# confluentinc/quickstart-streaming-agents

Measured on NVIDIA H100. Metric: rag_queries_per_sec_10Mx1536_top10, higher is better.
Workload: dtype bf16

## Files before the change

quickstart-streaming-agents_b200/csrc/sa_api.cu:

```cuda
#include "../../include/sa_api.h"
#include "sa_aux.cuh"
#include "sa_scan.cuh"

#include <cuda.h>
#include <cuda_runtime.h>
#include <dlfcn.h>
#include <nccl.h>

#include <algorithm>
#include <cstdarg>
#include <cstddef>
#include <cstdio>
#include <cstring>
#include <string>
#include <vector>

namespace {

thread_local char g_err[512] = "";

int fail(int rc, const char* fmt, ...) {
  va_list ap;
  va_start(ap, fmt);
  vsnprintf(g_err, sizeof g_err, fmt, ap);
// ... 278 lines not shown
    if (cg == 1 && kl == 16) return launch_scan<1, 16, sa::kModeProd, sa::kEpiSub>(tq, tc, p, grid, st);
    if (cg == 1 && kl == 32) return launch_scan<1, 32, sa::kModeProd, sa::kEpiSub>(tq, tc, p, grid, st);
    if (cg == 2 && kl == 16) return launch_scan<2, 16, sa::kModeProd, sa::kEpiSub>(tq, tc, p, grid, st);
    if (cg == 2 && kl == 32) return launch_scan<2, 32, sa::kModeProd, sa::kEpiSub>(tq, tc, p, grid, st);
    return fail(SA_ERR_ARG, "no scan instantiation for cta_group %d list %d", cg, kl);
  }
  if (mode == sa::kModeDots) {
    if (cg == 1) return launch_scan<1, 16, sa::kModeDots>(tq, tc, p, grid, st);
    return launch_scan<2, 16, sa::kModeDots>(tq, tc, p, grid, st);
  }
  if (mode == sa::kModeProf) {
    if (cg == 1 && kl == 16) return launch_scan<1, 16, sa::kModeProf>(tq, tc, p, grid, st);
    if (cg == 2 && kl == 16) return launch_scan<2, 16, sa::kModeProf>(tq, tc, p, grid, st);
    return fail(SA_ERR_ARG, "the profiling build of the scan exists for 16-entry lists only");
  }
  if (cg == 1 && kl == 16) return launch_scan<1, 16, sa::kModeProd>(tq, tc, p, grid, st);
  if (cg == 1 && kl == 32) return launch_scan<1, 32, sa::kModeProd>(tq, tc, p, grid, st);
  if (cg == 2 && kl == 16) return launch_scan<2, 16, sa::kModeProd>(tq, tc, p, grid, st);
  if (cg == 2 && kl == 32) return launch_scan<2, 32, sa::kModeProd>(tq, tc, p, grid, st);
  return fail(SA_ERR_ARG, "no scan instantiation for cta_group %d list %d", cg, kl);
}

int choose_cg(const sa_engine* e, int nq) {
  if (e->opt_cta_group == 1 || e->opt_cta_group == 2) return e->opt_cta_group;
  return nq > 128 ? 2 : 1;
}

bool is_pinned(const void* p) {
  cudaPointerAttributes a;
  if (cudaPointerGetAttributes(&a, p) != cudaSuccess) {
// ... 30 lines not shown
              const sa::Filter* filters = nullptr) {
  if (nq <= 0 || nq > e->max_batch) return fail(SA_ERR_CAPACITY, "nq %d outside [1, max_batch %d]", nq, e->max_batch);
  if (k <= 0 || k > e->max_k) return fail(SA_ERR_ARG, "k %d outside [1, max_k %d]", k, e->max_k);
  if (!q_bf16 || !out_score || !out_idx) return fail(SA_ERR_ARG, "null buffer");
  if (reinterpret_cast<uintptr_t>(q_bf16) % 16) return fail(SA_ERR_ARG, "query buffer must be 16-byte aligned");
  SA_ON_DEVICE(e->device);

  const int kl = e->opt_list_len ? e->opt_list_len : (k <= 16 ? 16 : 32);
  if (k > kl) return fail(SA_ERR_ARG, "k %d needs candidate lists longer than list_len %d", k, kl);
  const int64_t n_rows = e->n_rows;
  const int num_tiles = static_cast<int>((n_rows + sa::kBlockN - 1) / sa::kBlockN);
  const int cg = choose_cg(e, nq);
  std::vector<LaunchPlan> plan = plan_search(e->num_sms, e->opt_max_launch_qblocks, nq, cg, std::max(num_tiles, 1));
  if (static_cast<int>(plan.size()) > kMaxLaunches)
    return fail(SA_ERR_CAPACITY, "batch needs %zu scan launches (max %d)", plan.size(), kMaxLaunches);
  const int mode = e->opt_profile ? sa::kModeProf : sa::kModeProd;
  const int epi = (e->sim == SA_SIM_EUCLIDEAN ? sa::kEpiSub : sa::kEpiMul) | (filters != nullptr ? sa::kEpiFilt : 0);
  const float eps_rel = scan_eps_rel(e->dim);

  SA_CUDA(cudaStreamWaitEvent(st, e->scratch_free, 0));
  if (e->scratch_dirty) {
    int rc = zero_scan_scratch(e, st);
    if (rc) return rc;
    e->scratch_dirty = false;
  }
  sa_engine::Timing& tm = e->ring[e->n_searches % kTimingRing];
  tm.launches = 0;
  tm.kernels = 0;
  SA_CUDA(cudaEventRecord(tm.ev_total[0], st));
  e->scratch_dirty = true;
  int min_tl = sa::kMaxLanes;
// ... 162 lines not shown
  const double n = static_cast<double>(n_rows), d = e->dim, b = nq;
  tm.bytes = plan.size() * (n * d * 2.0 + n * 4.0) + b * d * 2.0 + b * k * 8.0;
  tm.flops = 2.0 * b * n * d;
  e->n_searches += 1;
  return SA_OK;
}

}

namespace {
template <int kKL>
void run_list(const float* score, const int32_t* row, int n, const float* floor_after, float* out_sc, int32_t* out_id,
              float* out_drop) {
  sa::TopList<kKL> L;
  L.init(nullptr);
  float ones[sa::kChunk];
  for (int j = 0; j < sa::kChunk; ++j) ones[j] = 1.0f;
  for (int c0 = 0; c0 < n; c0 += sa::kChunk) {
    float v[sa::kChunk];
    for (int j = 0; j < sa::kChunk; ++j) {
      const int i = c0 + j;
      v[j] = i < n ? score[i] : NAN;
      if (i < n && floor_after && floor_after[i] > -INFINITY) L.apply_shared(sa::float_to_key(floor_after[i]));
    }
    sa::chunk_process<kKL>(L, v, ones, c0);
  }
  for (int i = 0; i < kKL; ++i) {
    out_sc[i] = L.sc[i];
    out_id[i] = L.id[i] >= 0 ? row[L.id[i]] : -1;
  }
  if (out_drop) *out_drop = L.drop;
}
}

extern "C" {

static_assert(sizeof(sa_filter) == sizeof(sa::Filter) && offsetof(sa_filter, all_of) == offsetof(sa::Filter, all_of) &&
                  offsetof(sa_filter, none_of) == offsetof(sa::Filter, none_of) &&
                  offsetof(sa_filter, any_of) == offsetof(sa::Filter, any_of),
              "sa_filter and sa::Filter must share one layout");
// ... 951 lines not shown
  }
  if (!strcmp(name, "presample")) {
    if (value < -1 || value > 4096) return fail(SA_ERR_ARG, "presample must be in [-1, 4096]");
    e->opt_presample = static_cast<int>(value);
    return SA_OK;
  }
  if (!strcmp(name, "force_fix")) {
    e->opt_force_fix = value ? 1 : 0;
    return SA_OK;
  }
  if (!strcmp(name, "count_fix")) {
    e->opt_count_fix = value ? 1 : 0;
    return SA_OK;
  }
  if (!strcmp(name, "profile")) {
    e->opt_profile = value ? 1 : 0;
    return SA_OK;
  }
  if (!strcmp(name, "share_thresholds")) {
    e->opt_share_thresholds = value ? 1 : 0;
    return SA_OK;
  }
  if (!strcmp(name, "window_bound")) {
    e->opt_window_bound = value ? 1 : 0;
    return SA_OK;
  }
  if (!strcmp(name, "list_len")) {
    if (value != 0 && value != 16 && value != 32) return fail(SA_ERR_ARG, "list_len must be 0, 16 or 32");
    e->opt_list_len = static_cast<int>(value);
    return SA_OK;
  }
// ... 191 lines not shown
```

quickstart-streaming-agents_b200/csrc/sa_scan.cuh:

```cuda
#pragma once
#include "sa_aux.cuh"
#include "sm90_ptx.cuh"
#include <cmath>
#include <cstring>

namespace sa {

constexpr int kBlockM = 128;
constexpr int kBlockN = 256;
constexpr int kHalfN = kWgmmaN;
constexpr int kBlockK = 64;
constexpr int kUmmaK = 16;
constexpr int kScanThreads = 384;
constexpr int kProducerRegs = 40;
constexpr int kConsumerRegs = 232;
constexpr int kChunk = 32;
constexpr int kStagingLd = kHalfN + 4;
constexpr int kWin = 16;
constexpr int kWinWarmTiles = 16;

constexpr int kModeProd = 0;
constexpr int kModeDots = 1;
constexpr int kModeProf = 2;

constexpr int kEpiMul = 0;
constexpr int kEpiSub = 1;
constexpr int kEpiFilt = 2;

template <int kCG, bool kFilt = false>
struct ScanCfg {
  static constexpr int kStages = 3;
  static constexpr int kBRows = kBlockN / kCG;
  static constexpr uint32_t kABytes = kBlockM * kBlockK * 2;
  static constexpr uint32_t kBBytes = kBlockN * kBlockK * 2;
  static constexpr uint32_t kHalfBBytes = kHalfN * kBlockK * 2;
  static constexpr uint32_t kStageBytes = kABytes + kBBytes;
  static constexpr uint32_t kStagingBytes = kBlockM * kStagingLd * sizeof(float);
  static constexpr uint32_t kIcBytes = 4 * kBlockN * sizeof(float);
  static constexpr uint32_t kBarBytes = 2 * kStages * 8;
  static constexpr uint32_t kTagBytes = kFilt ? 4 * kBlockN * sizeof(unsigned long long) : 0;
  static constexpr uint32_t kSmemBytes = kStages * kStageBytes + kStagingBytes + kIcBytes + kBarBytes + kTagBytes + 1024;
  static_assert(kSmemBytes <= 227 * 1024, "H100 allows 227 KB of shared memory per block");
  static_assert(!kFilt || kSmemBytes == 228400, "filtered scan: the unfiltered 220 208 B plus 8 KB of tags");
};

struct ScanProf {
  long long prod_wait_empty;
  long long mma_wait_full;
  long long mma_wait_tempty;
  long long epi_wait_tfull;
  long long epi_busy;
  long long epi_slow_chunks;
  long long total;
  long long tiles;
};

struct ScanParams {
  const float* row_term;
// ... 138 lines not shown
      sc[i] = -INFINITY;
      id[i] = -1;
    }
    thr = thr_floor = published = drop = -INFINITY;
    nxt_key = 0u;
    slot = shared_slot;
  }
  __host__ __device__ __forceinline__ void apply_shared(unsigned key) {
    if (key != 0u) {
      thr_floor = max_nn(thr_floor, float_below(key_to_float(key)));
      thr = max_nn(thr, thr_floor);
    }
  }
};

template <int kKL, int kEpi = kEpiMul>
__host__ __device__ __forceinline__ bool chunk_process(TopList<kKL>& L, float (&v)[kChunk], const float (&w)[kChunk],
                                                       int row_base) {
  auto reduce = [&]() {
    float g[8];
#ifdef __CUDA_ARCH__
#pragma unroll
#endif
    for (int i = 0; i < 8; ++i)
      g[i] = max_nn(max_nn(v[4 * i + 0], v[4 * i + 1]), max_nn(v[4 * i + 2], v[4 * i + 3]));
    return max_nn(max_nn(max_nn(g[0], g[1]), max_nn(g[2], g[3])), max_nn(max_nn(g[4], g[5]), max_nn(g[6], g[7])));
  };
#ifdef __CUDA_ARCH__
#pragma unroll
#endif
  for (int i = 0; i < kChunk; ++i) {
    if constexpr (kEpi == kEpiSub)
      v[i] -= w[i];
    else
      v[i] *= w[i];
  }
  float m = reduce();
  if (!(m > L.thr)) {
    L.drop = max_nn(L.drop, m);
    return false;
  }
  do {
    int pos = kChunk - 1;
#ifdef __CUDA_ARCH__
#pragma unroll
#endif
    for (int j = kChunk - 2; j >= 0; --j) pos = (v[j] == m) ? j : pos;
    float sj = m;
    if (m == 0.f) {
#ifdef __CUDA_ARCH__
#pragma unroll
// ... 2 lines not shown
    }
#ifdef __CUDA_ARCH__
#pragma unroll
#endif
    for (int j = 0; j < kChunk; ++j) v[j] = (j == pos) ? -INFINITY : v[j];
    L.drop = max_nn(L.drop, L.sc[kKL - 1]);
    list_insert<kKL>(L.sc, L.id, sj, row_base + pos);
    L.thr = max_nn(L.sc[kKL - 1], L.thr_floor);
    m = reduce();
  } while (m > L.thr);
  L.drop = max_nn(L.drop, m);
  return true;
}

#ifdef __CUDACC__
template <int kKL, int kMode, int kEpi>
__device__ __forceinline__ int epilogue_half(TopList<kKL>& L, const float* srow, const float* ic, int row0,
                                             float* dbg_row, const unsigned long long* tg = nullptr,
                                             const Filter* fp = nullptr) {
  int slow = 0;
  float v[kChunk], w[kChunk];
#pragma unroll 1
  for (int c = 0; c < kHalfN / kChunk; ++c) {
    unsigned pass = 0u;
    if constexpr ((kEpi & kEpiFilt) != 0) {
      const Filter F = *fp;
#pragma unroll
      for (int j = 0; j < kChunk; ++j) pass |= filter_pass(tg[c * kChunk + j], F) ? (1u << j) : 0u;
    }
    const float4* s4 = reinterpret_cast<const float4*>(srow + c * kChunk);
    const float4* w4 = reinterpret_cast<const float4*>(ic + c * kChunk);
#pragma unroll
    for (int i = 0; i < kChunk / 4; ++i) {
      const float4 x = s4[i], y = w4[i];
      v[4 * i + 0] = x.x;
      v[4 * i + 1] = x.y;
      v[4 * i + 2] = x.z;
      v[4 * i + 3] = x.w;
      w[4 * i + 0] = y.x;
      w[4 * i + 1] = y.y;
      w[4 * i + 2] = y.z;
      w[4 * i + 3] = y.w;
    }
    if constexpr ((kEpi & kEpiFilt) != 0) {
      const float qnan = __int_as_float(0x7fc00000);
#pragma unroll
      for (int j = 0; j < kChunk; ++j) w[j] = ((pass >> j) & 1u) ? w[j] : qnan;
    }
    if constexpr (kMode == kModeDots) {
      if (dbg_row != nullptr) {
#pragma unroll
        for (int j = 0; j < kChunk; ++j) dbg_row[c * kChunk + j] = v[j];
      }
    }
    slow += chunk_process<kKL, kEpi & 1>(L, v, w, row0 + c * kChunk) ? 1 : 0;
    __syncwarp();
  }
  return slow;
}

template <int kCG, int kKL, int kMode, int kEpi = kEpiMul>
__global__ void __launch_bounds__(kScanThreads, 1)
sa_scan_kernel(const __grid_constant__ CUtensorMap tmap_q, const __grid_constant__ CUtensorMap tmap_c,
               const ScanParams p) {
  constexpr bool kFilt = (kEpi & kEpiFilt) != 0;
  using Cfg = ScanCfg<kCG, kFilt>;
  constexpr int kStages = Cfg::kStages;
  constexpr int kRowsPerQb = kBlockM * kCG;
  constexpr bool kProf = (kMode == kModeProf);

  extern __shared__ uint8_t smem_raw[];
  const uint32_t smem_base = (smem_u32(smem_raw) + 1023u) & ~1023u;
  uint8_t* smem_gen = smem_raw + (smem_base - smem_u32(smem_raw));

  float* staging = reinterpret_cast<float*>(smem_gen + kStages * Cfg::kStageBytes);
  float* icbuf = reinterpret_cast<float*>(smem_gen + kStages * Cfg::kStageBytes + Cfg::kStagingBytes);
  const uint32_t bar_base = smem_base + kStages * Cfg::kStageBytes + Cfg::kStagingBytes + Cfg::kIcBytes;
  auto full_bar = [&](int s) { return bar_base + 8u * s; };
  auto empty_bar = [&](int s) { return bar_base + 8u * (kStages + s); };
  auto a_smem = [&](int s) { return smem_base + s * Cfg::kStageBytes; };
  auto b_smem = [&](int s) { return smem_base + s * Cfg::kStageBytes + Cfg::kABytes; };
  const uint32_t tag_base = bar_base + Cfg::kBarBytes;

  const int warp = threadIdx.x >> 5;
  const int lane = threadIdx.x & 31;
  const uint32_t rank = (kCG == 2) ? cluster_ctarank() : 0u;
  const int TL = p.tl_count;
  const int nqb = p.nqb;
  struct Walk {
    int qb, tl, tiles;
  };
  auto walk_of = [&]() {
// ... 70 lines not shown
          }
        }
        if (lockstep) st_relaxed_gpu(p.lane_progress + tl * nqb + qb, tile_no + 1);
      }
      if constexpr (kProf) {
        p.prof[blockIdx.x].prod_wait_empty = waited;
        p.prof[blockIdx.x].tiles = tile_no;
      }
    }
  } else {
    setmaxnreg_inc<kConsumerRegs>();
    const Walk w = walk_of();
    const int qb = w.qb, tl = w.tl, walk_tiles = w.tiles;
    const int g = warp / 4 - 1;
    const int wt = threadIdx.x & 127;
    const bool epi = (warp & 3) < 2;
    const int ew = 2 * g + (warp & 3);
    const int et = 64 * g + wt;
    const bool signaller = wt == 0;
    const uint32_t named_bar = 1 + g;
    float* ic = icbuf + ew * kBlockN;
    float* stg = staging + 64 * g * kStagingLd;
    const int query = qb * kRowsPerQb + static_cast<int>(rank) * kBlockM + et;
    const bool own_query = epi && query < p.nq;
    TopList<kKL> L;
    L.init((p.thr_shared != nullptr && own_query) ? p.thr_shared + query : nullptr);

    constexpr float kPast = ((kEpi & 1) == kEpiSub) ? -1.f : 0.f;
    float4 nx0 = make_float4(0.f, 0.f, 0.f, 0.f), nx1 = nx0;
    auto fetch_ic = [&](int t) {
      const long long r0 = static_cast<long long>(t) * kBlockN + 8 * lane;
      const float4* src = reinterpret_cast<const float4*>(p.row_term + r0);
      if (r0 + 8 <= p.n_rows) {
        nx0 = __ldg(src);
        nx1 = __ldg(src + 1);
      } else {
        float x[8];
#pragma unroll
        for (int j = 0; j < 8; ++j) x[j] = (r0 + j < p.n_rows) ? __ldg(p.row_term + r0 + j) : kPast;
        nx0 = make_float4(x[0], x[1], x[2], x[3]);
        nx1 = make_float4(x[4], x[5], x[6], x[7]);
      }
    };
    if (epi && tl < walk_tiles) fetch_ic(tl * p.tile_stride);
    auto fetch_tags = [&](int t) {
      const long long r0 = static_cast<long long>(t) * kBlockN + 8 * lane;
      const uint32_t dst = tag_base + static_cast<uint32_t>((ew * kBlockN + 8 * lane) * sizeof(unsigned long long));
#pragma unroll
      for (int j = 0; j < 4; ++j) {
        const long long left = p.n_rows - (r0 + 2 * j);
        const uint32_t bytes = left >= 2 ? 16u : (left == 1 ? 8u : 0u);
        cp_async_16(dst + 16u * j, p.row_tags + (bytes != 0u ? r0 + 2 * j : 0), bytes);
      }
    };
    if constexpr (kFilt) {
      if (epi && tl < walk_tiles) fetch_tags(tl * p.tile_stride);
    }

    const bool win_on = p.lane2 != nullptr && TL >= kWin && own_query;
    const size_t win_stride = static_cast<size_t>(p.nqb) * kRowsPerQb;
    unsigned* const win_q = win_on ? p.lane2 + query : nullptr;
    float pub2 = -INFINITY;
    unsigned nx2[kWin] = {};
    bool have2 = false;

    const uint64_t a_desc0 = make_kmajor_sw128_desc(a_smem(0) + g * (64 * kBlockK * 2));
    const uint64_t b_desc0 = make_kmajor_sw128_desc(b_smem(0));
    constexpr uint64_t kStageDesc = Cfg::kStageBytes >> 4;
    constexpr uint64_t kHalfBDesc = Cfg::kHalfBBytes >> 4;
    int stage = 0;
    uint32_t phase = 0;
    long long w_full = 0, w_stage = 0, w_mma = 0, busy = 0, slow_chunks = 0;
    for (int ti = tl; ti < walk_tiles; ti += TL) {
      const int t = ti * p.tile_stride;
      int slow = 0;
      if (epi) {
        if (have2) {
          const unsigned kb = window_bound<kKL>(nx2);
          L.nxt_key = kb > L.nxt_key ? kb : L.nxt_key;
          have2 = false;
        }
        L.apply_shared(L.nxt_key);
        const float qnan = __int_as_float(0x7fc00000);
        auto sc = [&](float x) {
          if constexpr ((kEpi & 1) == kEpiSub)
            return x >= 0.f ? x : qnan;
          else
            return x > 0.f ? x : qnan;
        };
        float4* dst = reinterpret_cast<float4*>(ic + 8 * lane);
        dst[0] = make_float4(sc(nx0.x), sc(nx0.y), sc(nx0.z), sc(nx0.w));
        dst[1] = make_float4(sc(nx1.x), sc(nx1.y), sc(nx1.z), sc(nx1.w));
        __syncwarp();
      }
#pragma unroll
      for (int i = 0; i < kWin; ++i) nx2[i] = 0u;
      float* dbg_row = nullptr;
      if constexpr (kMode == kModeDots) {
        if (own_query && p.dbg_dots != nullptr && t == p.dbg_tile) dbg_row = p.dbg_dots + static_cast<size_t>(query) * kBlockN;
      }
      float acc0[64], acc1[64];
      int prev_stage = -1;
      for (int kb = 0; kb < p.num_kb; ++kb) {
        if constexpr (kProf) {
          const long long c0 = clock64();
          mbar_wait(full_bar(stage), phase, static_cast<uint32_t>(p.wait_hint_ns));
          w_full += clock64() - c0;
        } else {
          mbar_wait(full_bar(stage), phase, static_cast<uint32_t>(p.wait_hint_ns));
        }
        wgmma_fence();
        wgmma_fence_operands(acc0);
        wgmma_fence_operands(acc1);
#pragma unroll
        for (int k = 0; k < kBlockK / kUmmaK; ++k) {
          const uint64_t a_desc = a_desc0 + stage * kStageDesc + 2u * k;
          const uint64_t b_desc = b_desc0 + stage * kStageDesc + 2u * k;
          wgmma_m64n128k16_bf16(acc0, a_desc, b_desc, (kb | k) != 0 ? 1u : 0u);
          wgmma_m64n128k16_bf16(acc1, a_desc, b_desc + kHalfBDesc, (kb | k) != 0 ? 1u : 0u);
        }
        wgmma_commit();
        wgmma_fence_operands(acc0);
        wgmma_fence_operands(acc1);
        if (prev_stage >= 0) {
          wgmma_wait<1>();
          if (signaller) {
            mbar_arrive(empty_bar(prev_stage));
            if constexpr (kCG == 2) mbar_arrive_cluster(empty_bar(prev_stage), rank ^ 1u);
          }
        }
        prev_stage = stage;
        if (++stage == kStages) {
          stage = 0;
          phase ^= 1u;
        }
      }
      long long c0 = 0;
      if constexpr (kProf) c0 = clock64();
      wgmma_wait<0>();
      wgmma_fence_operands(acc0);
      wgmma_fence_operands(acc1);
      if (signaller) {
        mbar_arrive(empty_bar(prev_stage));
        if constexpr (kCG == 2) mbar_arrive_cluster(empty_bar(prev_stage), rank ^ 1u);
      }
      if constexpr (kProf) w_mma += clock64() - c0;
      if (epi && ti + TL < walk_tiles) fetch_ic((ti + TL) * p.tile_stride);
      auto stage_and_score = [&](const float (&acc)[64], int h) {
        long long c1 = 0;
        if constexpr (kProf) c1 = clock64();
        named_bar_sync(named_bar, 128);
#pragma unroll
        for (int j = 0; j < 16; ++j) {
          const int r = 16 * (wt >> 5) + ((wt & 31) >> 2);
          const int col = 8 * j + 2 * (wt & 3);
          *reinterpret_cast<float2*>(stg + r * kStagingLd + col) = make_float2(acc[4 * j + 0], acc[4 * j + 1]);
          *reinterpret_cast<float2*>(stg + (r + 8) * kStagingLd + col) = make_float2(acc[4 * j + 2], acc[4 * j + 3]);
        }
        named_bar_sync(named_bar, 128);
        long long c2 = 0;
        if constexpr (kProf) c2 = clock64();
        if constexpr (kFilt) {
          if (epi && h == 0) {
            cp_async_wait_all();
            __syncwarp();
          }
        }
        if constexpr (kFilt) {
          const unsigned long long* tg =
              reinterpret_cast<const unsigned long long*>(smem_gen + (tag_base - smem_base)) + ew * kBlockN;
          if (epi)
            slow += epilogue_half<kKL, kMode, kEpi>(L, stg + wt * kStagingLd, ic + h * kHalfN, t * kBlockN + h * kHalfN,
                                                    dbg_row != nullptr ? dbg_row + h * kHalfN : nullptr, tg + h * kHalfN,
                                                    p.filters + (own_query ? query : 0));
        } else if (epi) {
          slow += epilogue_half<kKL, kMode, kEpi>(L, stg + wt * kStagingLd, ic + h * kHalfN, t * kBlockN + h * kHalfN,
                                                  dbg_row != nullptr ? dbg_row + h * kHalfN : nullptr);
        }
        if constexpr (kProf) {
          w_stage += c2 - c1;
          busy += clock64() - c2;
        }
      };
      stage_and_score(acc0, 0);
      stage_and_score(acc1, 1);
      if constexpr (kFilt) {
        if (epi && ti + TL < walk_tiles) {
          __syncwarp();
          fetch_tags((ti + TL) * p.tile_stride);
        }
      }
      if constexpr (kProf) slow_chunks += slow;
      if (epi) {
        if (L.slot != nullptr) {
          if (L.sc[kKL - 1] > L.published) {
            L.published = L.sc[kKL - 1];
            atomicMax(L.slot, float_to_key(L.published));
          }
          L.nxt_key = ld_relaxed_gpu_u32(L.slot);
        }
        if (p.lane2 != nullptr && TL >= kWin) {
          const bool fetch = (ti - tl) / TL < kWinWarmTiles || __any_sync(0xffffffffu, slow > 0);
          if (win_on) {
            if (L.sc[1] > pub2) {
              pub2 = L.sc[1];
              st_relaxed_gpu_u32(win_q + static_cast<size_t>(tl) * win_stride, float_to_key(pub2));
            }
// ... 15 lines not shown

    if (own_query) {
      const size_t o = (static_cast<size_t>(blockIdx.x) * kBlockM + et) * kKL;
      float4* ps = reinterpret_cast<float4*>(p.part_score + o);
      int4* pi = reinterpret_cast<int4*>(p.part_idx + o);
#pragma unroll
      for (int i = 0; i < kKL / 4; ++i) {
        ps[i] = make_float4(L.sc[4 * i], L.sc[4 * i + 1], L.sc[4 * i + 2], L.sc[4 * i + 3]);
        pi[i] = make_int4(L.id[4 * i], L.id[4 * i + 1], L.id[4 * i + 2], L.id[4 * i + 3]);
      }
      p.part_drop[static_cast<size_t>(blockIdx.x) * kBlockM + et] = L.drop;
    }
    if constexpr (kProf) {
      if (g == 0 && signaller) {
        p.prof[blockIdx.x].mma_wait_full = w_full;
        p.prof[blockIdx.x].mma_wait_tempty = w_stage;
        p.prof[blockIdx.x].epi_wait_tfull = w_mma;
        p.prof[blockIdx.x].epi_busy = busy;
        p.prof[blockIdx.x].epi_slow_chunks = slow_chunks;
      }
    }
  }

  __syncthreads();
  if (p.dbg_times != nullptr && threadIdx.x == 0) p.dbg_times[2 * blockIdx.x + 1] = globaltimer_ns();
  if constexpr (kProf) {
    if (threadIdx.x == 0) p.prof[blockIdx.x].total = clock64() - t_start;
  }
  if constexpr (kCG == 2) cluster_sync_all();
}
#endif

}
```

quickstart-streaming-agents_b200/csrc/sm90_ptx.cuh:

```cuda
#pragma once
#include <cstdint>
#include <cuda.h>

namespace sa {

#ifndef SA_WATCHDOG_CYCLES
#define SA_WATCHDOG_CYCLES (4000000000ll)
#endif

__device__ __forceinline__ uint32_t smem_u32(const void* p) {
  return static_cast<uint32_t>(__cvta_generic_to_shared(p));
}
__device__ __forceinline__ uint32_t cluster_ctarank() {
  uint32_t r;
  asm volatile("mov.u32 %0, %%cluster_ctarank;" : "=r"(r));
  return r;
}

__device__ __forceinline__ void mbar_init(uint32_t bar, uint32_t count) {
  asm volatile("mbarrier.init.shared::cta.b64 [%0], %1;" ::"r"(bar), "r"(count) : "memory");
}
__device__ __forceinline__ void fence_mbar_init() {
  asm volatile("fence.mbarrier_init.release.cluster;" ::: "memory");
}
// ... 32 lines not shown
      : "r"(bar), "r"(parity), "r"(hint_ns)
      : "memory");
  return ok != 0;
}
__device__ __forceinline__ void mbar_wait(uint32_t bar, uint32_t parity, uint32_t hint_ns = 0) {
  if (mbar_try_wait(bar, parity)) return;
  const long long t0 = clock64();
  while (!(hint_ns ? mbar_try_wait_hint(bar, parity, hint_ns) : mbar_try_wait(bar, parity))) {
    if (clock64() - t0 > SA_WATCHDOG_CYCLES) __trap();
  }
}

__device__ __forceinline__ void named_bar_sync(uint32_t id, uint32_t nthreads) {
  asm volatile("bar.sync %0, %1;" ::"r"(id), "r"(nthreads) : "memory");
}

template <uint32_t N>
__device__ __forceinline__ void setmaxnreg_dec() {
  asm volatile("setmaxnreg.dec.sync.aligned.u32 %0;" ::"n"(N));
}
template <uint32_t N>
__device__ __forceinline__ void setmaxnreg_inc() {
  asm volatile("setmaxnreg.inc.sync.aligned.u32 %0;" ::"n"(N));
}

__device__ __forceinline__ long long globaltimer_ns() {
  long long t;
  asm volatile("mov.u64 %0, %%globaltimer;" : "=l"(t));
  return t;
}
// ... 45 lines not shown
      "cp.async.bulk.tensor.2d.shared::cluster.global.mbarrier::complete_tx::bytes.multicast::cluster.L2::cache_hint"
      " [%0], [%1, {%3, %4}], [%2], %5, %6;" ::"r"(dst),
      "l"(reinterpret_cast<uint64_t>(m)), "r"(bar), "r"(x), "r"(y), "h"(cta_mask), "l"(hint)
      : "memory");
}

__device__ __forceinline__ void wgmma_fence() { asm volatile("wgmma.fence.sync.aligned;" ::: "memory"); }
__device__ __forceinline__ void wgmma_commit() { asm volatile("wgmma.commit_group.sync.aligned;" ::: "memory"); }
template <int N>
__device__ __forceinline__ void wgmma_wait() {
  asm volatile("wgmma.wait_group.sync.aligned %0;" ::"n"(N) : "memory");
}

constexpr int kWgmmaN = 128;

__device__ __forceinline__ void wgmma_m64n128k16_bf16(float (&d)[64], uint64_t a_desc, uint64_t b_desc,
                                                      uint32_t accumulate) {
  asm volatile(
      "{\n\t.reg .pred p;\n\t"
      "setp.ne.b32 p, %66, 0;\n\t"
      "wgmma.mma_async.sync.aligned.m64n128k16.f32.bf16.bf16 "
      "{%0, %1, %2, %3, %4, %5, %6, %7, %8, %9, %10, %11, %12, %13, %14, %15, "
      "%16, %17, %18, %19, %20, %21, %22, %23, %24, %25, %26, %27, %28, %29, %30, %31, "
      "%32, %33, %34, %35, %36, %37, %38, %39, %40, %41, %42, %43, %44, %45, %46, %47, "
      "%48, %49, %50, %51, %52, %53, %54, %55, %56, %57, %58, %59, %60, %61, %62, %63}, "
      "%64, %65, p, 1, 1, 0, 0;\n\t}"
      : "+f"(d[0]), "+f"(d[1]), "+f"(d[2]), "+f"(d[3]), "+f"(d[4]), "+f"(d[5]), "+f"(d[6]), "+f"(d[7]),
        "+f"(d[8]), "+f"(d[9]), "+f"(d[10]), "+f"(d[11]), "+f"(d[12]), "+f"(d[13]), "+f"(d[14]), "+f"(d[15]),
        "+f"(d[16]), "+f"(d[17]), "+f"(d[18]), "+f"(d[19]), "+f"(d[20]), "+f"(d[21]), "+f"(d[22]), "+f"(d[23]),
        "+f"(d[24]), "+f"(d[25]), "+f"(d[26]), "+f"(d[27]), "+f"(d[28]), "+f"(d[29]), "+f"(d[30]), "+f"(d[31]),
        "+f"(d[32]), "+f"(d[33]), "+f"(d[34]), "+f"(d[35]), "+f"(d[36]), "+f"(d[37]), "+f"(d[38]), "+f"(d[39]),
        "+f"(d[40]), "+f"(d[41]), "+f"(d[42]), "+f"(d[43]), "+f"(d[44]), "+f"(d[45]), "+f"(d[46]), "+f"(d[47]),
        "+f"(d[48]), "+f"(d[49]), "+f"(d[50]), "+f"(d[51]), "+f"(d[52]), "+f"(d[53]), "+f"(d[54]), "+f"(d[55]),
        "+f"(d[56]), "+f"(d[57]), "+f"(d[58]), "+f"(d[59]), "+f"(d[60]), "+f"(d[61]), "+f"(d[62]), "+f"(d[63])
      : "l"(a_desc), "l"(b_desc), "r"(accumulate)
      : "memory");
}
__device__ __forceinline__ void wgmma_fence_operands(float (&d)[64]) {
#pragma unroll
  for (int i = 0; i < 64; ++i) asm volatile("" : "+f"(d[i])::"memory");
}

__device__ __forceinline__ uint64_t make_kmajor_sw128_desc(uint32_t smem_addr) {
  uint64_t d = 0;
  d |= static_cast<uint64_t>((smem_addr & 0x3FFFFu) >> 4);
  d |= static_cast<uint64_t>(1) << 16;
  d |= static_cast<uint64_t>(1024 >> 4) << 32;
  d |= static_cast<uint64_t>(1) << 62;
  return d;
}

}
```

Baseline: 13690.

## Score accumulator fragments in registers, staging only hot chunks, with 4 pipeline stages

```diff
diff --git a/quickstart-streaming-agents_b200/csrc/sa_api.cu b/quickstart-streaming-agents_b200/csrc/sa_api.cu
--- a/quickstart-streaming-agents_b200/csrc/sa_api.cu
+++ b/quickstart-streaming-agents_b200/csrc/sa_api.cu
@@ -316,6 +316,11 @@
     if (cg == 2 && kl == 16) return launch_scan<2, 16, sa::kModeProf>(tq, tc, p, grid, st);
     return fail(SA_ERR_ARG, "the profiling build of the scan exists for 16-entry lists only");
   }
+  if (mode == sa::kModeMma) {
+    if (cg == 1 && kl == 16) return launch_scan<1, 16, sa::kModeMma>(tq, tc, p, grid, st);
+    if (cg == 2 && kl == 16) return launch_scan<2, 16, sa::kModeMma>(tq, tc, p, grid, st);
+    return fail(SA_ERR_ARG, "the MMA-only build of the scan exists for 16-entry lists only");
+  }
   if (cg == 1 && kl == 16) return launch_scan<1, 16, sa::kModeProd>(tq, tc, p, grid, st);
   if (cg == 1 && kl == 32) return launch_scan<1, 32, sa::kModeProd>(tq, tc, p, grid, st);
   if (cg == 2 && kl == 16) return launch_scan<2, 16, sa::kModeProd>(tq, tc, p, grid, st);
@@ -376,7 +381,7 @@
   std::vector<LaunchPlan> plan = plan_search(e->num_sms, e->opt_max_launch_qblocks, nq, cg, std::max(num_tiles, 1));
   if (static_cast<int>(plan.size()) > kMaxLaunches)
     return fail(SA_ERR_CAPACITY, "batch needs %zu scan launches (max %d)", plan.size(), kMaxLaunches);
-  const int mode = e->opt_profile ? sa::kModeProf : sa::kModeProd;
+  const int mode = e->opt_profile == 2 ? sa::kModeMma : e->opt_profile ? sa::kModeProf : sa::kModeProd;
   const int epi = (e->sim == SA_SIM_EUCLIDEAN ? sa::kEpiSub : sa::kEpiMul) | (filters != nullptr ? sa::kEpiFilt : 0);
   const float eps_rel = scan_eps_rel(e->dim);
 
@@ -569,8 +574,6 @@
               float* out_drop) {
   sa::TopList<kKL> L;
   L.init(nullptr);
-  float ones[sa::kChunk];
-  for (int j = 0; j < sa::kChunk; ++j) ones[j] = 1.0f;
   for (int c0 = 0; c0 < n; c0 += sa::kChunk) {
     float v[sa::kChunk];
     for (int j = 0; j < sa::kChunk; ++j) {
@@ -578,7 +581,7 @@
       v[j] = i < n ? score[i] : NAN;
       if (i < n && floor_after && floor_after[i] > -INFINITY) L.apply_shared(sa::float_to_key(floor_after[i]));
     }
-    sa::chunk_process<kKL>(L, v, ones, c0);
+    sa::chunk_process<kKL>(L, v, c0);
   }
   for (int i = 0; i < kKL; ++i) {
     out_sc[i] = L.sc[i];
@@ -1560,7 +1563,7 @@
     return SA_OK;
   }
   if (!strcmp(name, "profile")) {
-    e->opt_profile = value ? 1 : 0;
+    e->opt_profile = value == 2 ? 2 : (value ? 1 : 0);
     return SA_OK;
   }
   if (!strcmp(name, "share_thresholds")) {
diff --git a/quickstart-streaming-agents_b200/csrc/sa_scan.cuh b/quickstart-streaming-agents_b200/csrc/sa_scan.cuh
--- a/quickstart-streaming-agents_b200/csrc/sa_scan.cuh
+++ b/quickstart-streaming-agents_b200/csrc/sa_scan.cuh
@@ -15,13 +15,14 @@
 constexpr int kProducerRegs = 40;
 constexpr int kConsumerRegs = 232;
 constexpr int kChunk = 32;
-constexpr int kStagingLd = kHalfN + 4;
+constexpr int kSlotLd = kChunk + 4;
 constexpr int kWin = 16;
 constexpr int kWinWarmTiles = 16;
 
 constexpr int kModeProd = 0;
 constexpr int kModeDots = 1;
 constexpr int kModeProf = 2;
+constexpr int kModeMma = 3;
 
 constexpr int kEpiMul = 0;
 constexpr int kEpiSub = 1;
@@ -29,19 +30,21 @@
 
 template <int kCG, bool kFilt = false>
 struct ScanCfg {
-  static constexpr int kStages = 3;
+  static constexpr int kStages = 4;
   static constexpr int kBRows = kBlockN / kCG;
   static constexpr uint32_t kABytes = kBlockM * kBlockK * 2;
   static constexpr uint32_t kBBytes = kBlockN * kBlockK * 2;
   static constexpr uint32_t kHalfBBytes = kHalfN * kBlockK * 2;
   static constexpr uint32_t kStageBytes = kABytes + kBBytes;
-  static constexpr uint32_t kStagingBytes = kBlockM * kStagingLd * sizeof(float);
-  static constexpr uint32_t kIcBytes = 4 * kBlockN * sizeof(float);
+  static constexpr uint32_t kIcBytes = 2 * kBlockN * sizeof(float);
+  static constexpr uint32_t kSlotBytes = kBlockM * kSlotLd * sizeof(float);
+  static constexpr uint32_t kQWordBytes = 3 * kBlockM * sizeof(float);
   static constexpr uint32_t kBarBytes = 2 * kStages * 8;
-  static constexpr uint32_t kTagBytes = kFilt ? 4 * kBlockN * sizeof(unsigned long long) : 0;
-  static constexpr uint32_t kSmemBytes = kStages * kStageBytes + kStagingBytes + kIcBytes + kBarBytes + kTagBytes + 1024;
+  static constexpr uint32_t kTagBytes = kFilt ? 2 * kBlockN * sizeof(unsigned long long) : 0;
+  static constexpr uint32_t kSmemBytes =
+      kStages * kStageBytes + kIcBytes + kSlotBytes + kQWordBytes + kBarBytes + kTagBytes + 1024;
   static_assert(kSmemBytes <= 227 * 1024, "H100 allows 227 KB of shared memory per block");
-  static_assert(!kFilt || kSmemBytes == 228400, "filtered scan: the unfiltered 220 208 B plus 8 KB of tags");
+  static_assert(!kFilt || kSmemBytes == 223808, "filtered scan: the unfiltered 219 712 B plus 4 KB of tags");
 };
 
 struct ScanProf {
@@ -210,9 +213,8 @@
   }
 };
 
-template <int kKL, int kEpi = kEpiMul>
-__host__ __device__ __forceinline__ bool chunk_process(TopList<kKL>& L, float (&v)[kChunk], const float (&w)[kChunk],
-                                                       int row_base) {
+template <int kKL>
+__host__ __device__ __forceinline__ bool chunk_process(TopList<kKL>& L, float (&v)[kChunk], int row_base) {
   auto reduce = [&]() {
     float g[8];
 #ifdef __CUDA_ARCH__
@@ -222,15 +224,6 @@
       g[i] = max_nn(max_nn(v[4 * i + 0], v[4 * i + 1]), max_nn(v[4 * i + 2], v[4 * i + 3]));
     return max_nn(max_nn(max_nn(g[0], g[1]), max_nn(g[2], g[3])), max_nn(max_nn(g[4], g[5]), max_nn(g[6], g[7])));
   };
-#ifdef __CUDA_ARCH__
-#pragma unroll
-#endif
-  for (int i = 0; i < kChunk; ++i) {
-    if constexpr (kEpi == kEpiSub)
-      v[i] -= w[i];
-    else
-      v[i] *= w[i];
-  }
   float m = reduce();
   if (!(m > L.thr)) {
     L.drop = max_nn(L.drop, m);
@@ -263,51 +256,6 @@
 }
 
 #ifdef __CUDACC__
-template <int kKL, int kMode, int kEpi>
-__device__ __forceinline__ int epilogue_half(TopList<kKL>& L, const float* srow, const float* ic, int row0,
-                                             float* dbg_row, const unsigned long long* tg = nullptr,
-                                             const Filter* fp = nullptr) {
-  int slow = 0;
-  float v[kChunk], w[kChunk];
-#pragma unroll 1
-  for (int c = 0; c < kHalfN / kChunk; ++c) {
-    unsigned pass = 0u;
-    if constexpr ((kEpi & kEpiFilt) != 0) {
-      const Filter F = *fp;
-#pragma unroll
-      for (int j = 0; j < kChunk; ++j) pass |= filter_pass(tg[c * kChunk + j], F) ? (1u << j) : 0u;
-    }
-    const float4* s4 = reinterpret_cast<const float4*>(srow + c * kChunk);
-    const float4* w4 = reinterpret_cast<const float4*>(ic + c * kChunk);
-#pragma unroll
-    for (int i = 0; i < kChunk / 4; ++i) {
-      const float4 x = s4[i], y = w4[i];
-      v[4 * i + 0] = x.x;
-      v[4 * i + 1] = x.y;
-      v[4 * i + 2] = x.z;
-      v[4 * i + 3] = x.w;
-      w[4 * i + 0] = y.x;
-      w[4 * i + 1] = y.y;
-      w[4 * i + 2] = y.z;
-      w[4 * i + 3] = y.w;
-    }
-    if constexpr ((kEpi & kEpiFilt) != 0) {
-      const float qnan = __int_as_float(0x7fc00000);
-#pragma unroll
-      for (int j = 0; j < kChunk; ++j) w[j] = ((pass >> j) & 1u) ? w[j] : qnan;
-    }
-    if constexpr (kMode == kModeDots) {
-      if (dbg_row != nullptr) {
-#pragma unroll
-        for (int j = 0; j < kChunk; ++j) dbg_row[c * kChunk + j] = v[j];
-      }
-    }
-    slow += chunk_process<kKL, kEpi & 1>(L, v, w, row0 + c * kChunk) ? 1 : 0;
-    __syncwarp();
-  }
-  return slow;
-}
-
 template <int kCG, int kKL, int kMode, int kEpi = kEpiMul>
 __global__ void __launch_bounds__(kScanThreads, 1)
 sa_scan_kernel(const __grid_constant__ CUtensorMap tmap_q, const __grid_constant__ CUtensorMap tmap_c,
@@ -316,15 +264,17 @@
   using Cfg = ScanCfg<kCG, kFilt>;
   constexpr int kStages = Cfg::kStages;
   constexpr int kRowsPerQb = kBlockM * kCG;
-  constexpr bool kProf = (kMode == kModeProf);
+  constexpr bool kMma = (kMode == kModeMma);
+  constexpr bool kProf = (kMode == kModeProf) || kMma;
 
   extern __shared__ uint8_t smem_raw[];
   const uint32_t smem_base = (smem_u32(smem_raw) + 1023u) & ~1023u;
   uint8_t* smem_gen = smem_raw + (smem_base - smem_u32(smem_raw));
 
-  float* staging = reinterpret_cast<float*>(smem_gen + kStages * Cfg::kStageBytes);
-  float* icbuf = reinterpret_cast<float*>(smem_gen + kStages * Cfg::kStageBytes + Cfg::kStagingBytes);
-  const uint32_t bar_base = smem_base + kStages * Cfg::kStageBytes + Cfg::kStagingBytes + Cfg::kIcBytes;
+  float* icbuf = reinterpret_cast<float*>(smem_gen + kStages * Cfg::kStageBytes);
+  float* slots = icbuf + 2 * kBlockN;
+  float* qwords = slots + kBlockM * kSlotLd;
+  const uint32_t bar_base = smem_base + kStages * Cfg::kStageBytes + Cfg::kIcBytes + Cfg::kSlotBytes + Cfg::kQWordBytes;
   auto full_bar = [&](int s) { return bar_base + 8u * s; };
   auto empty_bar = [&](int s) { return bar_base + 8u * (kStages + s); };
   auto a_smem = [&](int s) { return smem_base + s * Cfg::kStageBytes; };
@@ -425,47 +375,44 @@
     const int qb = w.qb, tl = w.tl, walk_tiles = w.tiles;
     const int g = warp / 4 - 1;
     const int wt = threadIdx.x & 127;
-    const bool epi = (warp & 3) < 2;
-    const int ew = 2 * g + (warp & 3);
+    const int quad = lane & 3;
+    const int fr = 16 * (wt >> 5) + (lane >> 2);
+    const bool epi = wt < 64;
     const int et = 64 * g + wt;
     const bool signaller = wt == 0;
     const uint32_t named_bar = 1 + g;
-    float* ic = icbuf + ew * kBlockN;
-    float* stg = staging + 64 * g * kStagingLd;
-    const int query = qb * kRowsPerQb + static_cast<int>(rank) * kBlockM + et;
+    float* ic = icbuf + g * kBlockN;
+    float* slot = slots + 64 * g * kSlotLd;
+    float* thr_s = qwords + 64 * g;
+    float* rej_s = qwords + kBlockM + 64 * g;
+    unsigned* hot_s = reinterpret_cast<unsigned*>(qwords + 2 * kBlockM) + 64 * g;
+    const int qrow0 = qb * kRowsPerQb + static_cast<int>(rank) * kBlockM + 64 * g;
+    const int query = qrow0 + wt;
     const bool own_query = epi && query < p.nq;
     TopList<kKL> L;
     L.init((p.thr_shared != nullptr && own_query) ? p.thr_shared + query : nullptr);
 
     constexpr float kPast = ((kEpi & 1) == kEpiSub) ? -1.f : 0.f;
-    float4 nx0 = make_float4(0.f, 0.f, 0.f, 0.f), nx1 = nx0;
+    float2 nx = make_float2(0.f, 0.f);
     auto fetch_ic = [&](int t) {
-      const long long r0 = static_cast<long long>(t) * kBlockN + 8 * lane;
-      const float4* src = reinterpret_cast<const float4*>(p.row_term + r0);
-      if (r0 + 8 <= p.n_rows) {
-        nx0 = __ldg(src);
-        nx1 = __ldg(src + 1);
+      const long long r0 = static_cast<long long>(t) * kBlockN + 2 * wt;
+      if (r0 + 2 <= p.n_rows) {
+        nx = __ldg(reinterpret_cast<const float2*>(p.row_term + r0));
       } else {
-        float x[8];
-#pragma unroll
-        for (int j = 0; j < 8; ++j) x[j] = (r0 + j < p.n_rows) ? __ldg(p.row_term + r0 + j) : kPast;
-        nx0 = make_float4(x[0], x[1], x[2], x[3]);
-        nx1 = make_float4(x[4], x[5], x[6], x[7]);
+        nx.x = r0 < p.n_rows ? __ldg(p.row_term + r0) : kPast;
+        nx.y = kPast;
       }
     };
-    if (epi && tl < walk_tiles) fetch_ic(tl * p.tile_stride);
+    if (!kMma && tl < walk_tiles) fetch_ic(tl * p.tile_stride);
     auto fetch_tags = [&](int t) {
-      const long long r0 = static_cast<long long>(t) * kBlockN + 8 * lane;
-      const uint32_t dst = tag_base + static_cast<uint32_t>((ew * kBlockN + 8 * lane) * sizeof(unsigned long long));
-#pragma unroll
-      for (int j = 0; j < 4; ++j) {
-        const long long left = p.n_rows - (r0 + 2 * j);
-        const uint32_t bytes = left >= 2 ? 16u : (left == 1 ? 8u : 0u);
-        cp_async_16(dst + 16u * j, p.row_tags + (bytes != 0u ? r0 + 2 * j : 0), bytes);
-      }
+      const long long r0 = static_cast<long long>(t) * kBlockN + 2 * wt;
+      const uint32_t dst = tag_base + static_cast<uint32_t>((g * kBlockN + 2 * wt) * sizeof(unsigned long long));
+      const long long left = p.n_rows - r0;
+      const uint32_t bytes = left >= 2 ? 16u : (left == 1 ? 8u : 0u);
+      cp_async_16(dst, p.row_tags + (bytes != 0u ? r0 : 0), bytes);
     };
     if constexpr (kFilt) {
-      if (epi && tl < walk_tiles) fetch_tags(tl * p.tile_stride);
+      if (tl < walk_tiles) fetch_tags(tl * p.tile_stride);
     }
 
     const bool win_on = p.lane2 != nullptr && TL >= kWin && own_query;
@@ -479,38 +426,34 @@
     const uint64_t b_desc0 = make_kmajor_sw128_desc(b_smem(0));
     constexpr uint64_t kStageDesc = Cfg::kStageBytes >> 4;
     constexpr uint64_t kHalfBDesc = Cfg::kHalfBBytes >> 4;
+    const float qnan = __int_as_float(0x7fc00000);
     int stage = 0;
     uint32_t phase = 0;
-    long long w_full = 0, w_stage = 0, w_mma = 0, busy = 0, slow_chunks = 0;
+    long long w_full = 0, w_open = 0, w_mma = 0, busy = 0, rounds_sum = 0;
     for (int ti = tl; ti < walk_tiles; ti += TL) {
       const int t = ti * p.tile_stride;
       int slow = 0;
-      if (epi) {
-        if (have2) {
-          const unsigned kb = window_bound<kKL>(nx2);
-          L.nxt_key = kb > L.nxt_key ? kb : L.nxt_key;
-          have2 = false;
-        }
-        L.apply_shared(L.nxt_key);
-        const float qnan = __int_as_float(0x7fc00000);
+      if constexpr (!kMma) {
+        if (epi) {
+          if (have2) {
+            const unsigned kb = window_bound<kKL>(nx2);
+            L.nxt_key = kb > L.nxt_key ? kb : L.nxt_key;
+            have2 = false;
+          }
+          L.apply_shared(L.nxt_key);
+          thr_s[wt] = L.thr;
+        }
         auto sc = [&](float x) {
           if constexpr ((kEpi & 1) == kEpiSub)
             return x >= 0.f ? x : qnan;
           else
             return x > 0.f ? x : qnan;
         };
-        float4* dst = reinterpret_cast<float4*>(ic + 8 * lane);
-        dst[0] = make_float4(sc(nx0.x), sc(nx0.y), sc(nx0.z), sc(nx0.w));
-        dst[1] = make_float4(sc(nx1.x), sc(nx1.y), sc(nx1.z), sc(nx1.w));
-        __syncwarp();
+        *reinterpret_cast<float2*>(ic + 2 * wt) = make_float2(sc(nx.x), sc(nx.y));
       }
 #pragma unroll
       for (int i = 0; i < kWin; ++i) nx2[i] = 0u;
-      float* dbg_row = nullptr;
-      if constexpr (kMode == kModeDots) {
-        if (own_query && p.dbg_dots != nullptr && t == p.dbg_tile) dbg_row = p.dbg_dots + static_cast<size_t>(query) * kBlockN;
-      }
-      float acc0[64], acc1[64];
+      float acc[128];
       int prev_stage = -1;
       for (int kb = 0; kb < p.num_kb; ++kb) {
         if constexpr (kProf) {
@@ -521,18 +464,16 @@
           mbar_wait(full_bar(stage), phase, static_cast<uint32_t>(p.wait_hint_ns));
         }
         wgmma_fence();
-        wgmma_fence_operands(acc0);
-        wgmma_fence_operands(acc1);
+        wgmma_fence_operands(acc);
 #pragma unroll
         for (int k = 0; k < kBlockK / kUmmaK; ++k) {
           const uint64_t a_desc = a_desc0 + stage * kStageDesc + 2u * k;
           const uint64_t b_desc = b_desc0 + stage * kStageDesc + 2u * k;
-          wgmma_m64n128k16_bf16(acc0, a_desc, b_desc, (kb | k) != 0 ? 1u : 0u);
-          wgmma_m64n128k16_bf16(acc1, a_desc, b_desc + kHalfBDesc, (kb | k) != 0 ? 1u : 0u);
+          wgmma_m64n128k16_bf16<0>(acc, a_desc, b_desc, (kb | k) != 0 ? 1u : 0u);
+          wgmma_m64n128k16_bf16<64>(acc, a_desc, b_desc + kHalfBDesc, (kb | k) != 0 ? 1u : 0u);
         }
         wgmma_commit();
-        wgmma_fence_operands(acc0);
-        wgmma_fence_operands(acc1);
+        wgmma_fence_operands(acc);
         if (prev_stage >= 0) {
           wgmma_wait<1>();
           if (signaller) {
@@ -549,59 +490,152 @@
       long long c0 = 0;
       if constexpr (kProf) c0 = clock64();
       wgmma_wait<0>();
-      wgmma_fence_operands(acc0);
-      wgmma_fence_operands(acc1);
+      wgmma_fence_operands(acc);
       if (signaller) {
         mbar_arrive(empty_bar(prev_stage));
         if constexpr (kCG == 2) mbar_arrive_cluster(empty_bar(prev_stage), rank ^ 1u);
       }
       if constexpr (kProf) w_mma += clock64() - c0;
-      if (epi && ti + TL < walk_tiles) fetch_ic((ti + TL) * p.tile_stride);
-      auto stage_and_score = [&](const float (&acc)[64], int h) {
-        long long c1 = 0;
-        if constexpr (kProf) c1 = clock64();
+      if constexpr (kMma) continue;
+      if (ti + TL < walk_tiles) fetch_ic((ti + TL) * p.tile_stride);
+
+      long long c1 = 0;
+      if constexpr (kProf) c1 = clock64();
+      if constexpr (kFilt) cp_async_wait_all();
+      named_bar_sync(named_bar, 128);
+      long long c2 = 0;
+      if constexpr (kProf) c2 = clock64();
+      if constexpr (kMode == kModeDots) {
+        if (p.dbg_dots != nullptr && t == p.dbg_tile) {
+#pragma unroll
+          for (int h = 0; h < 2; ++h) {
+            const int q = qrow0 + fr + 8 * h;
+            if (q < p.nq) {
+              float* drow = p.dbg_dots + static_cast<size_t>(q) * kBlockN + 2 * quad;
+#pragma unroll
+              for (int j = 0; j < 32; ++j)
+                *reinterpret_cast<float2*>(drow + 8 * j) = make_float2(acc[4 * j + 2 * h], acc[4 * j + 2 * h + 1]);
+            }
+          }
+        }
+      }
+      Filter f0, f1;
+      if constexpr (kFilt) {
+        const int q0 = qrow0 + fr, q1 = q0 + 8;
+        f0 = p.filters[q0 < p.nq ? q0 : 0];
+        f1 = p.filters[q1 < p.nq ? q1 : 0];
+      }
+      const unsigned long long* tg =
+          reinterpret_cast<const unsigned long long*>(smem_gen + (tag_base - smem_base)) + g * kBlockN;
+      const float thr0 = thr_s[fr], thr1 = thr_s[fr + 8];
+      float rej0 = -INFINITY, rej1 = -INFINITY;
+      unsigned hot = 0u;
+#pragma unroll
+      for (int c = 0; c < kBlockN / kChunk; ++c) {
+        float m0 = 0.f, m1 = 0.f;
+#pragma unroll
+        for (int jj = 0; jj < 4; ++jj) {
+          const int j = 4 * c + jj;
+          const int col = 8 * j + 2 * quad;
+          const float2 wv = *reinterpret_cast<const float2*>(ic + col);
+          float w00 = wv.x, w01 = wv.y, w10 = wv.x, w11 = wv.y;
+          if constexpr (kFilt) {
+            const ulonglong2 tt = *reinterpret_cast<const ulonglong2*>(tg + col);
+            w00 = filter_pass(tt.x, f0) ? w00 : qnan;
+            w01 = filter_pass(tt.y, f0) ? w01 : qnan;
+            w10 = filter_pass(tt.x, f1) ? w10 : qnan;
+            w11 = filter_pass(tt.y, f1) ? w11 : qnan;
+          }
+          if constexpr ((kEpi & 1) == kEpiSub) {
+            acc[4 * j + 0] -= w00;
+            acc[4 * j + 1] -= w01;
+            acc[4 * j + 2] -= w10;
+            acc[4 * j + 3] -= w11;
+          } else {
+            acc[4 * j + 0] *= w00;
+            acc[4 * j + 1] *= w01;
+            acc[4 * j + 2] *= w10;
+            acc[4 * j + 3] *= w11;
+          }
+          const float a0 = max_nn(acc[4 * j + 0], acc[4 * j + 1]), a1 = max_nn(acc[4 * j + 2], acc[4 * j + 3]);
+          m0 = jj == 0 ? a0 : max_nn(m0, a0);
+          m1 = jj == 0 ? a1 : max_nn(m1, a1);
+        }
+        m0 = max_nn(m0, __shfl_xor_sync(0xffffffffu, m0, 1));
+        m1 = max_nn(m1, __shfl_xor_sync(0xffffffffu, m1, 1));
+        m0 = max_nn(m0, __shfl_xor_sync(0xffffffffu, m0, 2));
+        m1 = max_nn(m1, __shfl_xor_sync(0xffffffffu, m1, 2));
+        if (m0 > thr0)
+          hot |= 1u << c;
+        else
+          rej0 = max_nn(rej0, m0);
+        if (m1 > thr1)
+          hot |= 1u << (8 + c);
+        else
+          rej1 = max_nn(rej1, m1);
+      }
+      if (quad == 0) {
+        rej_s[fr] = rej0;
+        rej_s[fr + 8] = rej1;
+        hot_s[fr] = hot & 0xffu;
+        hot_s[fr + 8] = hot >> 8;
+      }
+      auto put = [&]() {
+#pragma unroll
+        for (int h = 0; h < 2; ++h) {
+          const unsigned bits = (hot >> (8 * h)) & 0xffu;
+          const unsigned low = bits & (0u - bits);
+          float* dst = slot + (fr + 8 * h) * kSlotLd + 2 * quad;
+#pragma unroll
+          for (int c = 0; c < kBlockN / kChunk; ++c) {
+            if (low == (1u << c)) {
+#pragma unroll
+              for (int jj = 0; jj < 4; ++jj) {
+                const int j = 4 * c + jj;
+                *reinterpret_cast<float2*>(dst + 8 * jj) = make_float2(acc[4 * j + 2 * h], acc[4 * j + 2 * h + 1]);
+              }
+            }
+          }
+        }
+      };
+      put();
+      bool more = named_bar_any(named_bar, 128, hot != 0u);
+      unsigned own_hot = 0u;
+      if (epi) {
+        L.drop = max_nn(L.drop, rej_s[wt]);
+        own_hot = hot_s[wt];
+      }
+      int rounds = 0;
+      while (more) {
+        ++rounds;
+        if (own_hot != 0u) {
+          float v[kChunk];
+          const float4* s4 = reinterpret_cast<const float4*>(slot + wt * kSlotLd);
+#pragma unroll
+          for (int i = 0; i < kChunk / 4; ++i) {
+            const float4 x = s4[i];
+            v[4 * i + 0] = x.x;
+            v[4 * i + 1] = x.y;
+            v[4 * i + 2] = x.z;
+            v[4 * i + 3] = x.w;
+          }
+          slow += chunk_process<kKL>(L, v, t * kBlockN + (__ffs(own_hot) - 1) * kChunk) ? 1 : 0;
+          own_hot &= own_hot - 1u;
+        }
+        const unsigned b0 = hot & 0xffu, b1 = hot & 0xff00u;
+        hot &= ~((b0 & (0u - b0)) | (b1 & (0u - b1)));
         named_bar_sync(named_bar, 128);
-#pragma unroll
-        for (int j = 0; j < 16; ++j) {
-          const int r = 16 * (wt >> 5) + ((wt & 31) >> 2);
-          const int col = 8 * j + 2 * (wt & 3);
-          *reinterpret_cast<float2*>(stg + r * kStagingLd + col) = make_float2(acc[4 * j + 0], acc[4 * j + 1]);
-          *reinterpret_cast<float2*>(stg + (r + 8) * kStagingLd + col) = make_float2(acc[4 * j + 2], acc[4 * j + 3]);
-        }
-        named_bar_sync(named_bar, 128);
-        long long c2 = 0;
-        if constexpr (kProf) c2 = clock64();
-        if constexpr (kFilt) {
-          if (epi && h == 0) {
-            cp_async_wait_all();
-            __syncwarp();
-          }
-        }
-        if constexpr (kFilt) {
-          const unsigned long long* tg =
-              reinterpret_cast<const unsigned long long*>(smem_gen + (tag_base - smem_base)) + ew * kBlockN;
-          if (epi)
-            slow += epilogue_half<kKL, kMode, kEpi>(L, stg + wt * kStagingLd, ic + h * kHalfN, t * kBlockN + h * kHalfN,
-                                                    dbg_row != nullptr ? dbg_row + h * kHalfN : nullptr, tg + h * kHalfN,
-                                                    p.filters + (own_query ? query : 0));
-        } else if (epi) {
-          slow += epilogue_half<kKL, kMode, kEpi>(L, stg + wt * kStagingLd, ic + h * kHalfN, t * kBlockN + h * kHalfN,
-                                                  dbg_row != nullptr ? dbg_row + h * kHalfN : nullptr);
-        }
-        if constexpr (kProf) {
-          w_stage += c2 - c1;
-          busy += clock64() - c2;
-        }
-      };
-      stage_and_score(acc0, 0);
-      stage_and_score(acc1, 1);
+        put();
+        more = named_bar_any(named_bar, 128, hot != 0u);
+      }
       if constexpr (kFilt) {
-        if (epi && ti + TL < walk_tiles) {
-          __syncwarp();
-          fetch_tags((ti + TL) * p.tile_stride);
-        }
-      }
-      if constexpr (kProf) slow_chunks += slow;
+        if (ti + TL < walk_tiles) fetch_tags((ti + TL) * p.tile_stride);
+      }
+      if constexpr (kProf) {
+        w_open += c2 - c1;
+        busy += clock64() - c2;
+        rounds_sum += rounds;
+      }
       if (epi) {
         if (L.slot != nullptr) {
           if (L.sc[kKL - 1] > L.published) {
@@ -647,10 +681,10 @@
     if constexpr (kProf) {
       if (g == 0 && signaller) {
         p.prof[blockIdx.x].mma_wait_full = w_full;
-        p.prof[blockIdx.x].mma_wait_tempty = w_stage;
+        p.prof[blockIdx.x].mma_wait_tempty = w_open;
         p.prof[blockIdx.x].epi_wait_tfull = w_mma;
         p.prof[blockIdx.x].epi_busy = busy;
-        p.prof[blockIdx.x].epi_slow_chunks = slow_chunks;
+        p.prof[blockIdx.x].epi_slow_chunks = rounds_sum;
       }
     }
   }
diff --git a/quickstart-streaming-agents_b200/csrc/sm90_ptx.cuh b/quickstart-streaming-agents_b200/csrc/sm90_ptx.cuh
--- a/quickstart-streaming-agents_b200/csrc/sm90_ptx.cuh
+++ b/quickstart-streaming-agents_b200/csrc/sm90_ptx.cuh
@@ -70,6 +70,18 @@
 __device__ __forceinline__ void named_bar_sync(uint32_t id, uint32_t nthreads) {
   asm volatile("bar.sync %0, %1;" ::"r"(id), "r"(nthreads) : "memory");
 }
+__device__ __forceinline__ bool named_bar_any(uint32_t id, uint32_t nthreads, bool pred) {
+  uint32_t r;
+  asm volatile(
+      "{\n\t.reg .pred p, q;\n\t"
+      "setp.ne.u32 q, %3, 0;\n\t"
+      "bar.red.or.pred p, %1, %2, q;\n\t"
+      "selp.u32 %0, 1, 0, p;\n\t}"
+      : "=r"(r)
+      : "r"(id), "r"(nthreads), "r"(static_cast<uint32_t>(pred))
+      : "memory");
+  return r != 0;
+}
 
 template <uint32_t N>
 __device__ __forceinline__ void setmaxnreg_dec() {
@@ -145,31 +157,43 @@
 
 constexpr int kWgmmaN = 128;
 
-__device__ __forceinline__ void wgmma_m64n128k16_bf16(float (&d)[64], uint64_t a_desc, uint64_t b_desc,
+template <int kOff>
+__device__ __forceinline__ void wgmma_m64n128k16_bf16(float (&d)[128], uint64_t a_desc, uint64_t b_desc,
                                                       uint32_t accumulate) {
+  static_assert(kOff == 0 || kOff == 64, "one of the two 64-float halves of a 128-float accumulator set");
   asm volatile(
       "{\n\t.reg .pred p;\n\t"
       "setp.ne.b32 p, %66, 0;\n\t"
       "wgmma.mma_async.sync.aligned.m64n128k16.f32.bf16.bf16 "
-      "{%0, %1, %2, %3, %4, %5, %6, %7, %8, %9, %10, %11, %12, %13, %14, %15, "
+      "{"
+      "%0, %1, %2, %3, %4, %5, %6, %7, %8, %9, %10, %11, %12, %13, %14, %15, "
       "%16, %17, %18, %19, %20, %21, %22, %23, %24, %25, %26, %27, %28, %29, %30, %31, "
       "%32, %33, %34, %35, %36, %37, %38, %39, %40, %41, %42, %43, %44, %45, %46, %47, "
-      "%48, %49, %50, %51, %52, %53, %54, %55, %56, %57, %58, %59, %60, %61, %62, %63}, "
+      "%48, %49, %50, %51, %52, %53, %54, %55, %56, %57, %58, %59, %60, %61, %62, %63"
+      "}, "
       "%64, %65, p, 1, 1, 0, 0;\n\t}"
-      : "+f"(d[0]), "+f"(d[1]), "+f"(d[2]), "+f"(d[3]), "+f"(d[4]), "+f"(d[5]), "+f"(d[6]), "+f"(d[7]),
-        "+f"(d[8]), "+f"(d[9]), "+f"(d[10]), "+f"(d[11]), "+f"(d[12]), "+f"(d[13]), "+f"(d[14]), "+f"(d[15]),
-        "+f"(d[16]), "+f"(d[17]), "+f"(d[18]), "+f"(d[19]), "+f"(d[20]), "+f"(d[21]), "+f"(d[22]), "+f"(d[23]),
-        "+f"(d[24]), "+f"(d[25]), "+f"(d[26]), "+f"(d[27]), "+f"(d[28]), "+f"(d[29]), "+f"(d[30]), "+f"(d[31]),
-        "+f"(d[32]), "+f"(d[33]), "+f"(d[34]), "+f"(d[35]), "+f"(d[36]), "+f"(d[37]), "+f"(d[38]), "+f"(d[39]),
-        "+f"(d[40]), "+f"(d[41]), "+f"(d[42]), "+f"(d[43]), "+f"(d[44]), "+f"(d[45]), "+f"(d[46]), "+f"(d[47]),
-        "+f"(d[48]), "+f"(d[49]), "+f"(d[50]), "+f"(d[51]), "+f"(d[52]), "+f"(d[53]), "+f"(d[54]), "+f"(d[55]),
-        "+f"(d[56]), "+f"(d[57]), "+f"(d[58]), "+f"(d[59]), "+f"(d[60]), "+f"(d[61]), "+f"(d[62]), "+f"(d[63])
+      : "+f"(d[kOff + 0]), "+f"(d[kOff + 1]), "+f"(d[kOff + 2]), "+f"(d[kOff + 3]),
+        "+f"(d[kOff + 4]), "+f"(d[kOff + 5]), "+f"(d[kOff + 6]), "+f"(d[kOff + 7]),
+        "+f"(d[kOff + 8]), "+f"(d[kOff + 9]), "+f"(d[kOff + 10]), "+f"(d[kOff + 11]),
+        "+f"(d[kOff + 12]), "+f"(d[kOff + 13]), "+f"(d[kOff + 14]), "+f"(d[kOff + 15]),
+        "+f"(d[kOff + 16]), "+f"(d[kOff + 17]), "+f"(d[kOff + 18]), "+f"(d[kOff + 19]),
+        "+f"(d[kOff + 20]), "+f"(d[kOff + 21]), "+f"(d[kOff + 22]), "+f"(d[kOff + 23]),
+        "+f"(d[kOff + 24]), "+f"(d[kOff + 25]), "+f"(d[kOff + 26]), "+f"(d[kOff + 27]),
+        "+f"(d[kOff + 28]), "+f"(d[kOff + 29]), "+f"(d[kOff + 30]), "+f"(d[kOff + 31]),
+        "+f"(d[kOff + 32]), "+f"(d[kOff + 33]), "+f"(d[kOff + 34]), "+f"(d[kOff + 35]),
+        "+f"(d[kOff + 36]), "+f"(d[kOff + 37]), "+f"(d[kOff + 38]), "+f"(d[kOff + 39]),
+        "+f"(d[kOff + 40]), "+f"(d[kOff + 41]), "+f"(d[kOff + 42]), "+f"(d[kOff + 43]),
+        "+f"(d[kOff + 44]), "+f"(d[kOff + 45]), "+f"(d[kOff + 46]), "+f"(d[kOff + 47]),
+        "+f"(d[kOff + 48]), "+f"(d[kOff + 49]), "+f"(d[kOff + 50]), "+f"(d[kOff + 51]),
+        "+f"(d[kOff + 52]), "+f"(d[kOff + 53]), "+f"(d[kOff + 54]), "+f"(d[kOff + 55]),
+        "+f"(d[kOff + 56]), "+f"(d[kOff + 57]), "+f"(d[kOff + 58]), "+f"(d[kOff + 59]),
+        "+f"(d[kOff + 60]), "+f"(d[kOff + 61]), "+f"(d[kOff + 62]), "+f"(d[kOff + 63])
       : "l"(a_desc), "l"(b_desc), "r"(accumulate)
       : "memory");
 }
-__device__ __forceinline__ void wgmma_fence_operands(float (&d)[64]) {
+__device__ __forceinline__ void wgmma_fence_operands(float (&d)[128]) {
 #pragma unroll
-  for (int i = 0; i < 64; ++i) asm volatile("" : "+f"(d[i])::"memory");
+  for (int i = 0; i < 128; ++i) asm volatile("" : "+f"(d[i])::"memory");
 }
 
 __device__ __forceinline__ uint64_t make_kmajor_sw128_desc(uint32_t smem_addr) {
```

New measurement: 14660 (median of 6 runs). 1.07x the previous value.
